# cvg/pixel-perfect-sfm

Hardware: AMD Instinct MI355X
Metric: featuremetric residuals+Jacobians evaluated/sec (1M obs) (higher is better)
Workload: dtype f32 horizontal / f64 vertical+normalisation on f16 patches; 1 GPU; BASELINE.json configs[2]: synthetic 200 cams / 200000 points / 1000000 obs featuremetric BA residual+Jacobian evaluation, 128-ch fp16 16x16 patches, SIMPLE_RADIAL, fused six-scalar Jacobian reduction; n_obs=1000000, channels=128, patch=16, obs_per_gpu=1000000, partition=none

## Files before the change

### pixel-perfect-sfm_amd/csrc/pxr_ba_solve.hip

```cpp
#include <hip/hip_runtime.h>

#include <algorithm>
#include <chrono>
#include <cmath>
#include <cstdlib>
#include <cstring>
#include <limits>
#include <thread>
#include <vector>

#include "pxr_ba_pcg.h"
#include "pxr_ba_solve.h"
#include "pxr_device.h"
#include "pxr_internal.h"

namespace pxr {


constexpr int JAC_THREADS = 128;

__global__ __launch_bounds__(JAC_THREADS) void k_jac(const SolveDev d, const double* __restrict__ rec,
                                                     pxr_loss loss, double* __restrict__ L, double* __restrict__ W) {
  extern __shared__ double jstage[];
  const int lane = threadIdx.x & 63, wave = threadIdx.x >> 6;
  const int LS = d.LS, W3 = 3 * d.DC, WS = W3 + 1;
  double* Lw = jstage + (size_t)wave * 64 * (LS + WS);
  double* Ww = Lw + (size_t)64 * LS;
  const int64_t i0 = (int64_t)blockIdx.x * blockDim.x + wave * 64;
  const int64_t i = i0 + lane;
  const int n_valid = (int)min((int64_t)64, d.v.n_obs - i0);
  if (i < d.v.n_obs) {
  const int img = d.v.d_obs_image[i], pt = d.v.d_obs_point[i], cam = d.v.d_image_camera[img];
  double q[4], t[3], X[3], k[PXR_KPAD];
#pragma unroll
  for (int j = 0; j < 4; ++j) q[j] = d.v.d_qvec[4 * (size_t)img + j];
#pragma unroll
  for (int j = 0; j < 3; ++j) { t[j] = d.v.d_tvec[3 * (size_t)img + j]; X[j] = d.v.d_xyz[3 * (size_t)pt + j]; }
#pragma unroll
  for (int j = 0; j < PXR_KPAD; ++j) k[j] = d.v.d_cam_params[(size_t)cam * PXR_KPAD + j];
  const int model = d.v.d_cam_model[cam];
  double x, y, A[2][3], Pq[2][4], PX[2][3], Pk[2][PXR_KPAD];
  world_to_pixel_jac(model, k, q, t, X, x, y, A, Pq, PX, Pk);

  const double* r = rec + (size_t)i * PXR_OBS_REC;
  const double s = r[0], gxx = r[1], gxy = r[2], gyy = r[3], bx = r[4], by = r[5];
  double rho[3];
  loss_eval(loss.type, loss.a, 1.0, s, rho);
  double kappa = 0.0;
  if (s != 0.0 && rho[2] > 0.0) {
    const double D = 1.0 + 2.0 * s * rho[2] / rho[1];
    const double alpha = 1.0 - sqrt(D);
    kappa = (2.0 * alpha - alpha * alpha) / s;
  }
  double* Lo = Lw + (size_t)lane * LS;
  const double m00 = rho[1] * (gxx - kappa * bx * bx), m01 = rho[1] * (gxy - kappa * bx * by),
               m11 = rho[1] * (gyy - kappa * by * by);
  Lo[0] = m00; Lo[1] = m01; Lo[2] = m11;
  Lo[3] = rho[1] * bx;
  Lo[4] = rho[1] * by;
  const bool pvar = d.pt_var[pt] != 0;
  double e0[3], e1[3];
#pragma unroll
  for (int j = 0; j < 3; ++j) {
    const double sc = pvar ? d.scale_p[3 * (size_t)pt + j] : 0.0;
    e0[j] = PX[0][j] * sc; e1[j] = PX[1][j] * sc;
    Lo[5 + j] = e0[j];
    Lo[8 + j] = e1[j];
  }
  double me0[3], me1[3];
#pragma unroll
  for (int j = 0; j < 3; ++j) {
    me0[j] = m00 * e0[j] + m01 * e1[j];
    me1[j] = m01 * e0[j] + m11 * e1[j];
  }
  double* Wo = Ww + (size_t)lane * WS;
  double* B0 = Lo + 11;
  double* B1 = B0 + d.DC;
  int col = 0;
  auto put = [&](int c, double b0, double b1) {
    B0[c] = b0; B1[c] = b1;
    Wo[3 * c] = b0 * me0[0] + b1 * me1[0];
    Wo[3 * c + 1] = b0 * me0[1] + b1 * me1[1];
    Wo[3 * c + 2] = b0 * me0[2] + b1 * me1[2];
  };
  if (d.pose_dim[img] > 0) {
    const int po = d.pose_off[img];
    const double PJ[4][3] = {{-q[1], -q[2], -q[3]}, {q[0], q[3], -q[2]}, {-q[3], q[0], q[1]}, {q[2], -q[1], q[0]}};
#pragma unroll
    for (int a = 0; a < 3; ++a) {
      const double sc = d.scale_c[po + a];
      put(col, (Pq[0][0] * PJ[0][a] + Pq[0][1] * PJ[1][a] + Pq[0][2] * PJ[2][a] + Pq[0][3] * PJ[3][a]) * sc,
          (Pq[1][0] * PJ[0][a] + Pq[1][1] * PJ[1][a] + Pq[1][2] * PJ[2][a] + Pq[1][3] * PJ[3][a]) * sc);
      ++col;
    }
    const int tm = d.tmask[img];
#pragma unroll
    for (int a = 0; a < 3; ++a) {
      if ((tm >> a) & 1) continue;
      const double sc = d.scale_c[po + col];
      put(col, A[0][a] * sc, A[1][a] * sc);
      ++col;
    }
  }
  if (d.intr_dim[cam] > 0) {
    const int io = d.intr_off[cam], cm = d.cmask[cam], K = camera_num_params(model);
    int kc = 0;
#pragma unroll
    for (int a = 0; a < PXR_KPAD; ++a) {
      if (a >= K || ((cm >> a) & 1)) continue;
      const double sc = d.scale_c[io + kc];
      put(col, Pk[0][a] * sc, Pk[1][a] * sc);
      ++col; ++kc;
    }
  }
  for (; col < d.DC; ++col) put(col, 0.0, 0.0);
  }
  __threadfence_block();
  __builtin_amdgcn_wave_barrier();
  if (n_valid <= 0) return;
  double* Lg = L + (size_t)i0 * LS;
  for (int x = lane; x < n_valid * LS; x += 64) Lg[x] = Lw[x];
  double* Wg = W + (size_t)i0 * W3;
  for (int x = lane; x < n_valid * W3; x += 64) { const int o = x / W3; Wg[x] = Ww[o * WS + (x - o * W3)]; }
}

__global__ __launch_bounds__(256) void k_point(const SolveDev d, const int64_t* __restrict__ pt_ptr,
                                               const int64_t* __restrict__ pt_obs,
                                               const double* __restrict__ L, double* __restrict__ V,
                                               double* __restrict__ gp) {
  const int64_t p = (int64_t)blockIdx.x * blockDim.x + threadIdx.x;
  if (p >= d.v.n_points) return;
  double v[6] = {0, 0, 0, 0, 0, 0}, g[3] = {0, 0, 0};
  for (int64_t o = pt_ptr[p]; o < pt_ptr[p + 1]; ++o) {
    const double* Lo = L + (size_t)pt_obs[o] * d.LS;
    const double m00 = Lo[0], m01 = Lo[1], m11 = Lo[2], b0 = Lo[3], b1 = Lo[4];
    const double e0[3] = {Lo[5], Lo[6], Lo[7]}, e1[3] = {Lo[8], Lo[9], Lo[10]};
    double me0[3], me1[3];
#pragma unroll
    for (int j = 0; j < 3; ++j) { me0[j] = m00 * e0[j] + m01 * e1[j]; me1[j] = m01 * e0[j] + m11 * e1[j]; }
    v[0] += e0[0] * me0[0] + e1[0] * me1[0];
    v[1] += e0[0] * me0[1] + e1[0] * me1[1];
    v[2] += e0[0] * me0[2] + e1[0] * me1[2];
    v[3] += e0[1] * me0[1] + e1[1] * me1[1];
    v[4] += e0[1] * me0[2] + e1[1] * me1[2];
    v[5] += e0[2] * me0[2] + e1[2] * me1[2];
#pragma unroll
    for (int j = 0; j < 3; ++j) g[j] += e0[j] * b0 + e1[j] * b1;
  }
#pragma unroll
  for (int j = 0; j < 6; ++j) V[6 * p + j] = v[j];
#pragma unroll
  for (int j = 0; j < 3; ++j) gp[3 * p + j] = g[j];
}

constexpr int IMG_BATCH = 128;

__global__ __launch_bounds__(256) void k_img(const SolveDev d, const ImgChunk* __restrict__ chunks,
                                             const int64_t* __restrict__ img_obs,
                                             const double* __restrict__ L, double* __restrict__ U,
                                             double* __restrict__ gc, int block_form, double det_scale,
                                             double* __restrict__ chunk_trace, double* __restrict__ kpart, int ne_max) {
  extern __shared__ double stage[];
  const ImgChunk ch = chunks[blockIdx.x];
  const int img = ch.img, cam = d.v.d_image_camera[img];
  const int dc = d.pose_dim[img] + d.intr_dim[cam];
  if (dc == 0) { if (threadIdx.x == 0 && chunk_trace) chunk_trace[blockIdx.x] = 0.0; return; }
  const int LS = d.LS;
  double* red = stage + (size_t)IMG_BATCH * LS;
  const int NP = dc * (dc + 1) / 2, NE = NP + dc;
  const int slices = 256 / NE;
  const int e = threadIdx.x % NE, sl = threadIdx.x / NE;
  int a = 0, b = 0;
  const bool is_g = e >= NP;
  if (is_g) { a = e - NP; }
  else { int rem = e; a = 0; while (rem >= dc - a) { rem -= dc - a; ++a; } b = a + rem; }
  double acc = 0.0;
  long long qacc = 0;
  const bool fixed = det_scale != 0.0;
  constexpr int IMG_PF = 16;
  double pf[IMG_PF];
  auto request = [&](int64_t base) {
    const int nb = (int)min((int64_t)IMG_BATCH, ch.end - base);
#pragma unroll
    for (int j = 0; j < IMG_PF; ++j) {
      const int x = threadIdx.x + 256 * j;
      const int xc = min(x, nb * LS - 1);
      const int o = xc / LS, f = xc - o * LS;
      pf[j] = L[(size_t)img_obs[base + o] * LS + f];
    }
  };
  if (LS <= 2 * IMG_PF) {
    if (ch.begin < ch.end) request(ch.begin);
    for (int64_t base = ch.begin; base < ch.end; base += IMG_BATCH) {
      const int nb = (int)min((int64_t)IMG_BATCH, ch.end - base);
#pragma unroll
      for (int j = 0; j < IMG_PF; ++j) { const int x = threadIdx.x + 256 * j; if (x < nb * LS) stage[x] = pf[j]; }
      __syncthreads();
      if (base + IMG_BATCH < ch.end) request(base + IMG_BATCH);
      if (sl < slices) {
        for (int o = sl; o < nb; o += slices) {
          const double* Lo = stage + (size_t)o * LS;
          const double* B0 = Lo + 11; const double* B1 = B0 + d.DC;
          const double term = is_g ? B0[a] * Lo[3] + B1[a] * Lo[4]
                                   : B0[a] * (Lo[0] * B0[b] + Lo[1] * B1[b]) + B1[a] * (Lo[1] * B0[b] + Lo[2] * B1[b]);
          acc += term;
          if (fixed) qacc += __double2ll_rn(term * det_scale);
        }
      }
      __syncthreads();
    }
  } else {
  for (int64_t base = ch.begin; base < ch.end; base += IMG_BATCH) {
    const int nb = (int)min((int64_t)IMG_BATCH, ch.end - base);
    for (int x = threadIdx.x; x < nb * LS; x += 256) {
      const int o = x / LS, f = x - o * LS;
      stage[x] = L[(size_t)img_obs[base + o] * LS + f];
    }
    __syncthreads();
    if (sl < slices) {
      for (int o = sl; o < nb; o += slices) {
        const double* Lo = stage + (size_t)o * LS;
        const double* B0 = Lo + 11; const double* B1 = B0 + d.DC;
        const double term = is_g ? B0[a] * Lo[3] + B1[a] * Lo[4]
                                 : B0[a] * (Lo[0] * B0[b] + Lo[1] * B1[b]) + B1[a] * (Lo[1] * B0[b] + Lo[2] * B1[b]);
        acc += term;
        if (fixed) qacc += __double2ll_rn(term * det_scale);
      }
    }
    __syncthreads();
  }
  }
  red[threadIdx.x] = acc;
  __syncthreads();
  if (sl == 0) for (int s2 = 1; s2 < slices; ++s2) acc += red[s2 * NE + e];
  if (fixed) {
    __syncthreads();
    red[threadIdx.x] = __longlong_as_double(qacc);
    __syncthreads();
    if (sl == 0) for (int s2 = 1; s2 < slices; ++s2) qacc += __double_as_longlong(red[s2 * NE + e]);
    __syncthreads();
    red[threadIdx.x] = (sl == 0 && !is_g && a == b) ? acc : 0.0;
    __syncthreads();
    if (threadIdx.x == 0 && chunk_trace) {
      double tr = 0.0;
      for (int x = 0; x < NP; ++x) tr += red[x];
      chunk_trace[blockIdx.x] = tr;
    }
  }
  if (sl == 0 && kpart) {
    kpart[(size_t)blockIdx.x * ne_max + e] = acc;
  } else if (sl == 0) {
    const int ra = col_index(d, img, cam, a);
    const double v = fixed ? __longlong_as_double(qacc) : acc;
    if (is_g) accum_flush(gc + ra, v, det_scale);
    else if (block_form) {
      double* Ub = U + (size_t)img * d.DC * d.DC;
      accum_flush(Ub + a * d.DC + b, v, det_scale);
      if (a != b) accum_flush(Ub + b * d.DC + a, v, det_scale);
    } else accum_flush(U + (size_t)ra * d.n_c + col_index(d, img, cam, b), v, det_scale);
  }
}

__global__ __launch_bounds__(256) void k_pinv(int64_t n_points, const int* __restrict__ pt_var,
                                              const double* __restrict__ V,
                                              const double* __restrict__ Vdiag0 ,
                                              double inv_radius, double* __restrict__ T,
                                              double* __restrict__ zero_ptr, int zero_n) {
  if (blockIdx.x == 0) for (int e = threadIdx.x; e < zero_n; e += blockDim.x) zero_ptr[e] = 0.0;
  const int64_t p = (int64_t)blockIdx.x * blockDim.x + threadIdx.x;
  if (p >= n_points) return;
  double* To = T + 6 * p;
  if (!pt_var[p]) { for (int j = 0; j < 6; ++j) To[j] = 0.0; return; }
  const double a00 = V[6 * p] + Vdiag0[3 * p] * inv_radius, a01 = V[6 * p + 1], a02 = V[6 * p + 2];
  const double a11 = V[6 * p + 3] + Vdiag0[3 * p + 1] * inv_radius, a12 = V[6 * p + 4];
  const double a22 = V[6 * p + 5] + Vdiag0[3 * p + 2] * inv_radius;
  const double c00 = a11 * a22 - a12 * a12, c01 = a02 * a12 - a01 * a22, c02 = a01 * a12 - a02 * a11;
  const double det = a00 * c00 + a01 * c01 + a02 * c02;
  const double id = 1.0 / det;
  To[0] = c00 * id; To[1] = c01 * id; To[2] = c02 * id;
  To[3] = (a00 * a22 - a02 * a02) * id; To[4] = (a01 * a02 - a00 * a12) * id;
  To[5] = (a00 * a11 - a01 * a01) * id;
}

struct Copy4 { const double* src[4]; double* dst[4]; int64_t n[4]; };
__global__ __launch_bounds__(256) void k_copy4(const Copy4 c) {
  const int64_t stride = (int64_t)gridDim.x * blockDim.x, t0 = (int64_t)blockIdx.x * blockDim.x + threadIdx.x;
#pragma unroll
  for (int a = 0; a < 4; ++a)
    for (int64_t e = t0; e < c.n[a]; e += stride) c.dst[a][e] = c.src[a][e];
}

__global__ __launch_bounds__(256) void k_schur(const SolveDev d, const int64_t* __restrict__ pt_ptr,
                                               const int64_t* __restrict__ pt_obs,
                                               const double* __restrict__ W, const double* __restrict__ T,
                                               const double* __restrict__ gp, double* __restrict__ S,
                                               double* __restrict__ rhs, double det_scale) {
  const int64_t tid = (int64_t)blockIdx.x * blockDim.x + threadIdx.x;
  const int64_t i = tid / d.DC;
  const int a = (int)(tid - i * d.DC);
  if (i >= d.v.n_obs) return;
  const int img = d.v.d_obs_image[i], cam = d.v.d_image_camera[img];
  const int dci = d.pose_dim[img] + d.intr_dim[cam];
  if (a >= dci) return;
  const int pt = d.v.d_obs_point[i];
  if (!d.pt_var[pt]) return;
  double y0, y1, y2;
  y_row(W, T, i, a, d.DC, pt, y0, y1, y2);
  const int r = col_index(d, img, cam, a);
  accum_add(rhs + (size_t)r * d.ldS, -(y0 * gp[3 * (size_t)pt] + y1 * gp[3 * (size_t)pt + 1] + y2 * gp[3 * (size_t)pt + 2]), det_scale);
  for (int64_t o = pt_ptr[pt]; o < pt_ptr[pt + 1]; ++o) {
    const int64_t j = pt_obs[o];
    const int imgj = d.v.d_obs_image[j], camj = d.v.d_image_camera[imgj];
    const int dcj = d.pose_dim[imgj] + d.intr_dim[camj];
    const double* Wj = W + (size_t)j * d.DC * 3;
    for (int b = 0; b < dcj; ++b) {
      const int c = col_index(d, imgj, camj, b);
      if (r > c) continue;
      accum_add(S + (size_t)r * d.ldS + c, -(y0 * Wj[3 * b] + y1 * Wj[3 * b + 1] + y2 * Wj[3 * b + 2]), det_scale);
    }
  }
}

template <int G>
__global__ __launch_bounds__(1024) void k_schur_lds(const SolveDev d, const ImgChunk* __restrict__ chunks,
                                                    const int4* __restrict__ so,
                                                    const int* __restrict__ pj,
                                                    const int4* __restrict__ pcols,
                                                    const double* __restrict__ W, const double* __restrict__ T,
                                                    const double* __restrict__ gp, int CT,
                                                    double* __restrict__ S, double* __restrict__ rhs, double det_scale) {
  extern __shared__ double acc[];
  const ImgChunk ch = chunks[blockIdx.x];
  const int img = ch.img, cam = d.v.d_image_camera[img];
  const int dci = d.pose_dim[img] + d.intr_dim[cam];
  if (dci == 0) return;
  const int c0 = blockIdx.y * CT, c1 = min(d.n_c, c0 + CT);
  double* racc = acc + (size_t)d.DC * CT;
  double* ybuf = racc + d.DC;
  for (int e = threadIdx.x; e < dci * CT + d.DC; e += blockDim.x) {
    if (e < dci * CT) acc[(e / CT) * CT + (e % CT)] = 0.0; else racc[e - dci * CT] = 0.0;
  }
  __syncthreads();
  const int lane_b = threadIdx.x % G, grp = threadIdx.x / G, n_grp = blockDim.x / G;
  int rrow[G];
#pragma unroll
  for (int a = 0; a < G; ++a) rrow[a] = a < dci ? col_index(d, img, cam, a) : 0x7fffffff;
  constexpr int PB = 8;
  const bool first_tile = blockIdx.y == 0;
  int64_t o = ch.begin + grp;
  int4 s = o < ch.end ? so[o] : make_int4(0, 0, 0, 0);
  while (o < ch.end) {
    const int64_t o_next = o + n_grp;
    const int4 s_next = o_next < ch.end ? so[o_next] : make_int4(0, 0, 0, 0);
    if (s.w != 0) {
      const int64_t i = s.x, pt = s.y;
      const bool row_ok = lane_b < dci;
      const double* Wi = W + ((size_t)i * d.DC + (row_ok ? lane_b : 0)) * 3;
      const double* Tp = T + 6 * (size_t)pt;
      const double* gpp = gp + 3 * (size_t)pt;
      const double w0 = Wi[0], w1 = Wi[1], w2 = Wi[2];
      const double t0 = Tp[0], t1 = Tp[1], t2 = Tp[2], t3 = Tp[3], t4 = Tp[4], t5 = Tp[5];
      const double g0 = gpp[0], g1 = gpp[1], g2 = gpp[2];
      double y0 = 0.0, y1 = 0.0, y2 = 0.0;
      for (int kb = 0; kb < s.w; kb += PB) {
        int jj[PB];
        int4 cc[PB];
#pragma unroll
        for (int u = 0; u < PB; ++u) {
          const int idx = s.z + min(kb + u, s.w - 1);
          jj[u] = pj[idx]; cc[u] = pcols[idx];
        }
        double mm[PB][3];
        int col[PB];
#pragma unroll
        for (int u = 0; u < PB; ++u) {
          const int pdj = cc[u].y, dcj = pdj + cc[u].w;
          const bool has = kb + u < s.w && lane_b < dcj;
          const double* Wj = W + ((size_t)jj[u] * d.DC + (has ? lane_b : 0)) * 3;
          mm[u][0] = Wj[0]; mm[u][1] = Wj[1]; mm[u][2] = Wj[2];
          const int c = lane_b < pdj ? cc[u].x + lane_b : cc[u].z + (lane_b - pdj);
          col[u] = (has && c >= c0 && c < c1) ? c : -1;
        }
        if (kb == 0) {
          if (row_ok) { y0 = w0 * t0 + w1 * t1 + w2 * t2; y1 = w0 * t1 + w1 * t3 + w2 * t4; y2 = w0 * t2 + w1 * t4 + w2 * t5; }
          if (first_tile && row_ok) accum_add(racc + lane_b, -(y0 * g0 + y1 * g1 + y2 * g2), det_scale);
          double* yb = ybuf + 3 * (size_t)threadIdx.x;
          yb[0] = y0; yb[1] = y1; yb[2] = y2;
        }
        const double* yg = ybuf + 3 * (size_t)(threadIdx.x - lane_b);
#pragma unroll
        for (int a = 0; a < G; ++a) {
          const double ya0 = yg[3 * a], ya1 = yg[3 * a + 1], ya2 = yg[3 * a + 2];
#pragma unroll
          for (int u = 0; u < PB; ++u) {
            const int c = col[u];
            if (c >= 0 && c >= rrow[a])
              accum_add(acc + (size_t)a * CT + (c - c0), -(ya0 * mm[u][0] + ya1 * mm[u][1] + ya2 * mm[u][2]), det_scale);
          }
        }
      }
    }
    o = o_next; s = s_next;
  }
  __syncthreads();
  for (int e = threadIdx.x; e < dci * CT; e += blockDim.x) {
    const int a = e / CT, cl = e % CT;
    const double v = acc[(size_t)a * CT + cl];
    if (__double_as_longlong(v) != 0ll) accum_flush(S + (size_t)col_index(d, img, cam, a) * d.ldS + (c0 + cl), v, det_scale);
  }
  if (blockIdx.y == 0 && threadIdx.x < dci) {
    const double v = racc[threadIdx.x];
    if (__double_as_longlong(v) != 0ll) accum_flush(rhs + (size_t)col_index(d, img, cam, threadIdx.x) * d.ldS, v, det_scale);
  }
}

__global__ void k_copy_upper_add_diag(int n, const double* __restrict__ U, const double* __restrict__ damp,
                                      double inv_radius, const double* __restrict__ gc, double* __restrict__ S,
                                      int add_u, double det_scale) {
  const int64_t t = (int64_t)blockIdx.x * blockDim.x + threadIdx.x;
  const int ld = n + 1;
  if (t >= (int64_t)n * ld) return;
  const int r = (int)(t / ld), c = (int)(t % ld);
  double v = S[t];
  if (add_u) {
    v = (c < n && r <= c) ? U[(size_t)r * n + c] : 0.0;
  }
  else {
    if (det_scale != 0.0) v = (double)__double_as_longlong(v) / det_scale;
    if (r == c) v += damp[r] * inv_radius;
    if (c == n) v += gc[r];
  }
  S[t] = v;
}

__global__ void k_extract_diag(int n, const double* __restrict__ U, double* __restrict__ out) {
  const int i = blockIdx.x * blockDim.x + threadIdx.x;
  if (i < n) out[i] = U[(size_t)i * n + i];
}

__global__ void k_clamp(int64_t n, const double* __restrict__ in, double lo, double hi, double* __restrict__ out) {
  const int64_t i = (int64_t)blockIdx.x * blockDim.x + threadIdx.x;
  if (i < n) out[i] = fmin(fmax(in[i], lo), hi);
}

__global__ void k_point_diag(int64_t n_points, const double* __restrict__ V, double* __restrict__ out) {
  const int64_t p = (int64_t)blockIdx.x * blockDim.x + threadIdx.x;
  if (p >= n_points) return;
  out[3 * p] = V[6 * p]; out[3 * p + 1] = V[6 * p + 3]; out[3 * p + 2] = V[6 * p + 5];
}

__global__ void k_jacobi_scale(int64_t n, const double* __restrict__ diag, double* __restrict__ scale) {
  const int64_t i = (int64_t)blockIdx.x * blockDim.x + threadIdx.x;
  if (i < n) scale[i] = 1.0 / (1.0 + sqrt(diag[i]));
}

__global__ void k_axpy1(int n, const double* __restrict__ x, double* __restrict__ y) {
  const int i = blockIdx.x * blockDim.x + threadIdx.x;
  if (i < n) y[i] += x[i];
}

__global__ void k_fill(int64_t n, double v, double* __restrict__ out) {
  const int64_t i = (int64_t)blockIdx.x * blockDim.x + threadIdx.x;
  if (i < n) out[i] = v;
}

__global__ void k_finish_camera_step(int n, const double* __restrict__ x, const double* __restrict__ gc,
                                     const double* __restrict__ damp, double inv_radius,
                                     double* __restrict__ delta_c, double* __restrict__ scal_rep, long long* __restrict__ limb) {
  __shared__ long long lsh[PXR_LIMBS * 4];
  const int i = blockIdx.x * blockDim.x + threadIdx.x;
  double part = 0.0;
  if (i < n) {
    const double dl = -x[i];
    delta_c[i] = dl;
    part = dl * (damp[i] * inv_radius * dl - gc[i]);
  }
  if (limb) {
    Limbs l;
    if (i < n) l.add(part);
    limbs_block_add(l, limb + (8 + 0) * PXR_LIMBS, lsh);
// ... 799 lines not shown
    if (ctx->rank != 0) hipLaunchKernelGGL(k_zero, dim3(nblk(count)), dim3(256), 0, st, count, buf);
    return ar(buf, count);
  };
  struct { long long* p; } slimb;
  slimb.p = reinterpret_cast<long long*>(scal.p + 16);
  long long* const limb_arg = det ? slimb.p : nullptr;
  DevBuf<double> i64_halves;
  const bool native_i64 = allreduce == nullptr;
  if (det && multi && !native_i64) RC(i64_halves.alloc((size_t)2 * std::max<int64_t>({packed_doubles, 2 * (int64_t)nc1 + 8, 16 * PXR_LIMBS})));
  auto ar_i64 = [&](long long* buf, int64_t count) -> int {
    if (!multi || count <= 0) return PXR_OK;
    if (native_i64) return comm_allreduce_sum_i64(ctx, buf, count);
    hipLaunchKernelGGL(k_i64_split, dim3(nblk(count)), dim3(256), 0, st, count, (const long long*)buf, i64_halves.p);
    RC(ar(i64_halves.p, 2 * count));
    hipLaunchKernelGGL(k_i64_join, dim3(nblk(count)), dim3(256), 0, st, count, (const double*)i64_halves.p, buf);
    return PXR_OK;
  };
  auto zero_scalars = [&]() -> int {
    PXR_HIP(hipMemsetAsync(scal.p, 0, sizeof(double) * (16 + 16 * PXR_LIMBS + 1), st));
    return PXR_OK;
  };
  struct { double* p; } lin_stats;
  constexpr int kScalAll = 16 + 16 * PXR_LIMBS + 1 + 4;
  lin_stats.p = scal.p + (kScalAll - 4);
  if (!ctx->h_readback) PXR_HIP(hipHostMalloc(&ctx->h_readback, 4096, hipHostMallocDefault));
  static_assert(sizeof(double) * kScalAll <= 4096, "read-back buffer");
  double* const h_scal = static_cast<double*>(ctx->h_readback);
  std::memset(h_scal, 0, sizeof(double) * kScalAll);
  double* const h_lin_stats = h_scal + (kScalAll - 4);
  const int* const h_info_word = reinterpret_cast<const int*>(h_scal + 16 + 16 * PXR_LIMBS);
  const bool spin_wait = std::getenv("PXR_BLOCKING_WAIT") == nullptr;
  auto read_scal = [&](double* h16) -> int {
    if (det) {
      RC(ar_i64(slimb.p, 8 * PXR_LIMBS));
      hipLaunchKernelGGL(k_limbs_finish, dim3(1), dim3(64), 0, st, (const long long*)slimb.p, 0xffffu, scal.p);
    } else {
      hipLaunchKernelGGL(k_limbs_finish, dim3(1), dim3(64), 0, st, (const long long*)slimb.p, (1u << 0) | (1u << 4), scal.p);
      RC(ar(scal_sum, 8));
      RC(from_rank0(scal_rep, 8));
    }
    PXR_HIP(hipMemcpyAsync(h_scal, scal.p, sizeof(double) * kScalAll, hipMemcpyDeviceToHost, st));
    if (spin_wait) {
      PXR_HIP(hipEventRecord(ctx->ev_sync, st));
      hipError_t q;
      while ((q = hipEventQuery(ctx->ev_sync)) == hipErrorNotReady) {}
      PXR_HIP(q);
    } else PXR_HIP(hipStreamSynchronize(st));
    std::memcpy(h16, h_scal, sizeof(double) * 16);
    return PXR_OK;
  };
  DevBuf<double> det_part, chunk_trace;
  RC(det_part.alloc((size_t)n_pts + 8));
  RC(chunk_trace.alloc(chunks.size() + 1));
  auto det_scale_for = [](double md, double cost_now) {
    const double bound = 8.0 * std::max({md, std::sqrt(2.0 * md * std::max(cost_now, 0.0)), 1e-300});
    return std::ldexp(1.0, 62 - (int)std::ceil(std::log2(bound)));
  };
  double lin_md = 1.0;
  bool gram_cache = !geom && ctx->gram_cache && gram_eval_supported(arena, view) && cfg->use_float_simd == 0;
  bool gram_inner = !geom && opt->use_inner_iterations != 0 && arena->dtype != PXR_F64 && (arena->C == 128 || arena->C == 64) && !getenv("PXR_INNER_OLD") &&
                    !getenv("PXR_INNER_PACKED") && cfg->use_float_simd == 0;
  for (int c = 0; c < n_cam; ++c) gram_inner = gram_inner && cam_model[c] <= PXR_OPENCV;
  bool inner_cache = gram_inner && gram_eval_supported(arena, view) && !getenv("PXR_INNER_NO_CACHE");
  GramCache gram;
  if ((gram_cache || inner_cache) && gram_eval_prepare(ctx, arena, view, &gram) != PXR_OK) {
    gram_cache = false; inner_cache = false;
    (void)set_error(PXR_OK, "");
  }
  bool geom_ext = false;
  for (int c = 0; c < n_cam; ++c) geom_ext = geom_ext || cam_model[c] > PXR_OPENCV;
  setup_mark("Gram-matrix cache prepared");
  bool gram_warm = false;
  int n_evaluations = 0;
  bool cur_is_exact = true;
  auto evaluate = [&](const pxr_ba_view& v, double* rec) -> int {
    if (geom) RC(geom_eval(ctx, &v, d_obs_xy, rec, nullptr));
    else if (gram_cache && n_evaluations > 0) { RC(gram_evaluate(ctx, arena, &v, cfg, gram, rec)); gram_warm = true; }
    else RC(ba_eval_with_cost(ctx, arena, &v, cfg, 1, rec, nullptr, nullptr, nullptr, nullptr, nullptr));
    ++n_evaluations;
    hipLaunchKernelGGL(k_cost_limbs, dim3(1024), dim3(256), 0, st, (const double*)rec, n_obs, *loss, slimb.p + 0 * PXR_LIMBS);
    LAUNCH_CHECK("cost");
    return PXR_OK;
  };
  double lin_scale = 0.0;
  auto linearize = [&](const double* rec) -> int {
    hipLaunchKernelGGL(k_jac, dim3((unsigned)((n_obs + JAC_THREADS - 1) / JAC_THREADS)), dim3(JAC_THREADS),
                       sizeof(double) * (JAC_THREADS / 64) * 64 * (LS + 3 * DC + 1), st, dv, rec, *loss, L.p, W.p);
    hipLaunchKernelGGL(k_point, dim3(nblk(n_pts)), dim3(256), 0, st, dv, d_pt_ptr.p, d_pt_obs.p, L.p, V.p, gp.p);
    PXR_HIP(hipMemsetAsync(U.p, 0, sizeof(double) * U.n, st));
    PXR_HIP(hipMemsetAsync(gcd.p, 0, sizeof(double) * gcd.n, st));
    if (n_c > 0 && !chunks.empty()) {
      hipLaunchKernelGGL(k_img, dim3((unsigned)chunks.size()), dim3(256), sizeof(double) * ((size_t)IMG_BATCH * LS + 256), st, dv,
                         d_chunks.p, d_img_obs.p, L.p, U.p, gc, iterative ? 1 : 0, lin_scale, lin_scale != 0.0 ? chunk_trace.p : (double*)nullptr,
                         det_iter ? det_kpart.p : (double*)nullptr, det_ne_max);
      if (det_iter) {
        RC(pcg_blocks_from_partials(st, dv, d_kchunk_ptr.p, det_kpart.p, det_ne_max, U.p, det_gimg.p, d_col_ent_ptr.p, d_col_ent.p, diagU, gc));
        LAUNCH_CHECK("linearize kernels");
        RC(ar(gcd.p, 2 * (int64_t)nc1));
        return PXR_OK;
      }
      if (lin_scale != 0.0) {
        hipLaunchKernelGGL(k_diag_and_trace, dim3(1), dim3(1024), 0, st, n_c, (const double*)U.p, diagU, (const double*)chunk_trace.p, (int)chunks.size(),
                           reinterpret_cast<long long*>(gcd.p + 2 * nc1));
        RC(ar_i64(reinterpret_cast<long long*>(gcd.p), 2 * (int64_t)nc1 + PXR_LIMBS));
        hipLaunchKernelGGL(k_finish_and_stats, dim3(1), dim3(1024), 0, st, n_c, 2 * (int)nc1, gcd.p, lin_scale,
                           reinterpret_cast<const long long*>(gcd.p + 2 * nc1), lin_stats.p);
        LAUNCH_CHECK("linearize kernels");
        return PXR_OK;
      }
      if (iterative) RC(pcg_diag_from_blocks(st, dv, U.p, diagU));
      else hipLaunchKernelGGL(k_extract_diag, dim3(nblk(n_c)), dim3(256), 0, st, n_c, U.p, diagU);
    }
    LAUNCH_CHECK("linearize kernels");
    RC(ar(gcd.p, 2 * (int64_t)nc1));
    return PXR_OK;
  };
  auto lin_fits = [&](const double* stt, double md_made_for) {
    if (n_c == 0 || chunks.empty()) return true;
    const double mx = stt[0], sm = stt[1], mn = stt[2], tr = stt[3];
    if (!(std::isfinite(mx) && std::isfinite(sm) && std::isfinite(tr))) return false;
    if (mn < 0.0) return false;
    if (std::fabs(tr - sm) > std::ldexp(1.0, 61) / lin_scale) return false;
    return mx <= 8.0 * md_made_for;
  };
  bool lin_not_finite = false;
  auto linearize_checked = [&](const double* rec, double md_guess, double cost_now, bool refine = false) -> int {
    if (!det_fixed) return linearize(rec);
    for (int attempt = 0; attempt < 8; ++attempt) {
      lin_md = md_guess;
      lin_scale = det_scale_for(lin_md, cost_now);
      RC(linearize(rec));
      PXR_HIP(hipMemcpyAsync(h_lin_stats, lin_stats.p, sizeof(double) * 4, hipMemcpyDeviceToHost, st));
      PXR_HIP(hipStreamSynchronize(st));
      if (lin_fits(h_lin_stats, lin_md)) {
        if (refine && attempt == 0 && h_lin_stats[0] * 64.0 < md_guess) { md_guess = std::max(h_lin_stats[0], 1e-300); continue; }
        return PXR_OK;
      }
      if (!(std::isfinite(h_lin_stats[3]) && h_lin_stats[3] >= 0.0)) { lin_not_finite = true; return PXR_OK; }
      md_guess = std::max(h_lin_stats[3], 2.0 * md_guess);
    }
    return set_error(PXR_EINVAL, "pxr_ba_solve: the fixed-point grid of the deterministic mode could not be fitted");
  };
  auto refresh_damping = [&]() -> int {
    if (n_c > 0) hipLaunchKernelGGL(k_clamp, dim3(nblk(n_c)), dim3(256), 0, st, (int64_t)n_c, diagU, opt->min_lm_diagonal, opt->max_lm_diagonal, damp_c.p);
    hipLaunchKernelGGL(k_point_diag, dim3(nblk(n_pts)), dim3(256), 0, st, n_pts, V.p, Vd0.p);
    hipLaunchKernelGGL(k_clamp, dim3(nblk(n_pts * 3)), dim3(256), 0, st, n_pts * 3, Vd0.p, opt->min_lm_diagonal, opt->max_lm_diagonal, Vd0.p);
    LAUNCH_CHECK("damping kernels");
    return PXR_OK;
  };

  if (iterative) {
    pcg.st = st; pcg.dv = dv;
    pcg.chunks = d_schur_chunks.p; pcg.n_chunks = (int)schur_chunks.size(); pcg.so = d_so.p;
    pcg.pt_ptr = d_pt_ptr.p; pcg.part_obs = d_part_obs.p; pcg.obs_cols = d_obs_cols.p;
    pcg.W = W.p; pcg.T = T.p; pcg.gp = gp.p; pcg.gc = gc; pcg.damp_c = damp_c.p; pcg.Ublk = U.p;
    pcg.n_groups = (int)group_size.size(); pcg.col_group = d_col_group.p; pcg.group_size = d_group_size.p;
    pcg.group_cols = d_group_cols.p;
    pcg.u = pcg_u.p; pcg.Mloc = pcg_mloc.p; pcg.Gm = pcg_g.p;
    pcg.x = xsol.p; pcg.r = pcg_vec.p; pcg.p = pcg_vec.p + nc1; pcg.q = pcg_vec.p + 2 * nc1; pcg.z = pcg_vec.p + 3 * nc1;
    pcg.b = pcg_vec.p + 4 * nc1; pcg.cgs = pcg_scal.p; pcg.cg_part = pcg_scal.p + 16; pcg.d_fail = d_info;
    pcg.det = det_iter;
    if (det_iter) {
      pcg.chunk_ptr = d_schunk_ptr.p; pcg.col_ent_ptr = d_col_ent_ptr.p; pcg.col_ent = d_col_ent.p;
      pcg.wpart = det_wpart.p; pcg.mpart = det_mpart.p;
    }
  }
  const std::function<int(double*, int64_t)> ar_fn = ar;
  auto gradient_below_tolerance = [&](bool* below) -> int {
    double h[16];
    RC(zero_scalars());
    if (n_c > 0) hipLaunchKernelGGL(k_count_above, dim3(nblk(n_c)), dim3(256), 0, st, (int64_t)n_c, gc, scale_c.p, opt->gradient_tolerance, scal_rep + 4,
                                    det ? slimb.p + (8 + 4) * PXR_LIMBS : (long long*)nullptr);
    hipLaunchKernelGGL(k_count_above, dim3(nblk(n_pts * 3)), dim3(256), 0, st, n_pts * 3, gp.p, scale_p.p, opt->gradient_tolerance, scal_sum + 5,
                       det ? slimb.p + 5 * PXR_LIMBS : (long long*)nullptr);
    RC(read_scal(h));
    *below = h[5] == 0.0 && h[12] == 0.0;
    return PXR_OK;
  };

  struct InnerListsOwner { InnerLists l; ~InnerListsOwner() { free_inner_lists(&l); } } inner_lists;
  if (gram_inner) {
    const int64_t* h_pt_ptr = pt_cnt.data();
    std::vector<int64_t> pageable;
    void* wave_stage = nullptr;
    const size_t ptr_bytes = (sizeof(int64_t) * ((size_t)n_pts + 1) + 255) & ~(size_t)255, wave_bytes = inner_wave_stage_bytes(n_pts);
    if (device_lists) {
      int64_t* stage = (ptr_bytes + wave_bytes) <= ((size_t)1 << 28) ? static_cast<int64_t*>(setup_staging(ctx, ptr_bytes + wave_bytes)) : nullptr;
      if (stage) wave_stage = reinterpret_cast<char*>(stage) + ptr_bytes;
      else { pageable.resize((size_t)n_pts + 1); stage = pageable.data(); }
      PXR_HIP(hipMemcpyAsync(stage, d_pt_ptr.p, sizeof(int64_t) * ((size_t)n_pts + 1), hipMemcpyDeviceToHost, st));
      PXR_HIP(hipStreamSynchronize(st));
      h_pt_ptr = stage;
    }
    RC(make_inner_lists(ctx, h_pt_ptr, n_pts, wave_stage, wave_stage ? wave_bytes : 0, view, d_pt_ptr.p, d_pt_obs.p, &inner_lists.l));
  }
  setup_mark("inner-iteration tables");
  const auto t_loop0 = std::chrono::steady_clock::now();
  sum->setup_ms = std::chrono::duration<double, std::milli>(t_loop0 - t_setup0).count();
  sum->num_camera_unknowns = n_c; sum->num_point_unknowns = 3 * n_pvar;
  sum->iterations = 0; sum->num_successful = 0; sum->termination = PXR_TERM_NO_CONVERGENCE;
  const bool use_lds_schur = std::getenv("PXR_SCHUR_GLOBAL_ATOMICS") == nullptr;
  int CT = n_c > 0 ? std::min(n_c, (int)((128 * 1024 / 8 - DC) / DC)) : 1;
  int n_ctiles = n_c > 0 ? (n_c + CT - 1) / CT : 1;
  if (const char* e = std::getenv("PXR_SCHUR_CTILES")) n_ctiles = std::max(n_ctiles, std::min(std::max(1, n_c), std::atoi(e)));
  CT = n_c > 0 ? (n_c + n_ctiles - 1) / n_ctiles : 1;
  const size_t schur_shmem = sizeof(double) * ((size_t)DC * CT + DC + 3 * 1024);
  if (use_lds_schur && n_c > 0)
    PXR_HIP(hipFuncSetAttribute(reinterpret_cast<const void*>(DC <= 8 ? k_schur_lds<8> : (DC <= 16 ? k_schur_lds<16> : k_schur_lds<32>)),
                                hipFuncAttributeMaxDynamicSharedMemorySize, (int)schur_shmem));
  PXR_HIP(hipFuncSetAttribute(reinterpret_cast<const void*>(k_jac), hipFuncAttributeMaxDynamicSharedMemorySize,
                              (int)(sizeof(double) * (JAC_THREADS / 64) * 64 * (LS + 3 * DC + 1))));
  const bool verbose = std::getenv("PXR_VERBOSE") != nullptr;
  const bool phase_timing = std::getenv("PXR_PHASE_TIMING") != nullptr;
  double ph_ms[8] = {0, 0, 0, 0, 0, 0, 0, 0};
  auto ph_t0 = std::chrono::steady_clock::now();
  auto phase = [&](int k) {
    if (!phase_timing) return;
    (void)hipStreamSynchronize(st);
    const auto now = std::chrono::steady_clock::now();
    ph_ms[k] += std::chrono::duration<double, std::milli>(now - ph_t0).count();
    ph_t0 = now;
  };

  double hs[16];
  double* rec_cur = rec_a.p; double* rec_cand = rec_b.p;
  RC(zero_scalars());
  RC(evaluate(dv.v, rec_cur));
  RC(read_scal(hs));
  double cost = hs[0];
  sum->initial_cost = cost;
  if (!std::isfinite(cost)) {
    sum->final_cost = cost; sum->termination = PXR_TERM_FAILURE;
    sum->total_ms = std::chrono::duration<double, std::milli>(std::chrono::steady_clock::now() - t_loop0).count();
    return PXR_OK;
  }
  hipLaunchKernelGGL(k_fill, dim3(nblk(nc1)), dim3(256), 0, st, (int64_t)nc1, 1.0, scale_c.p);
  hipLaunchKernelGGL(k_fill, dim3(nblk(n_pts * 3)), dim3(256), 0, st, n_pts * 3, 1.0, scale_p.p);
  RC(linearize_checked(rec_cur, std::ldexp(1.0, 32), cost, !opt->jacobi_scaling));
  auto fail_not_finite = [&]() -> int {
    sum->final_cost = cost; sum->final_radius = opt->initial_radius; sum->termination = PXR_TERM_FAILURE;
    sum->total_ms = std::chrono::duration<double, std::milli>(std::chrono::steady_clock::now() - t_loop0).count();
    return PXR_OK;
  };
  if (lin_not_finite) return fail_not_finite();
  if (opt->jacobi_scaling) {
    if (n_c > 0) hipLaunchKernelGGL(k_jacobi_scale, dim3(nblk(n_c)), dim3(256), 0, st, (int64_t)n_c, diagU, scale_c.p);
    hipLaunchKernelGGL(k_point_diag, dim3(nblk(n_pts)), dim3(256), 0, st, n_pts, V.p, Vd0.p);
    hipLaunchKernelGGL(k_jacobi_scale, dim3(nblk(n_pts * 3)), dim3(256), 0, st, n_pts * 3, Vd0.p, scale_p.p);
    RC(linearize_checked(rec_cur, 1.0 / 8.0, cost));
    if (lin_not_finite) return fail_not_finite();
  }
  if (opt->gradient_tolerance > 0.0) {
    bool below = false;
    RC(gradient_below_tolerance(&below));
    if (below) {
      sum->termination = PXR_TERM_CONVERGENCE; sum->final_cost = cost; sum->final_radius = opt->initial_radius;
      sum->total_ms = std::chrono::duration<double, std::milli>(std::chrono::steady_clock::now() - t_loop0).count();
      return PXR_OK;
    }
  }
  double radius = opt->initial_radius, decrease_factor = 2.0;
  int invalid = 0;
  bool reuse_diag = false;
  bool inner_enabled = opt->use_inner_iterations != 0, inner_useful = false;
  PXR_HIP(hipStreamSynchronize(st));
  sum->initial_us = (int32_t)std::min<double>(2e9, 1e3 * std::chrono::duration<double, std::milli>(std::chrono::steady_clock::now() - t_loop0).count());
  bool any_cb = ctx->iter_cb != nullptr;
  if (multi) {
    double h = any_cb ? 1.0 : 0.0;
    PXR_HIP(hipMemcpyAsync(cb_flags.p, &h, sizeof(h), hipMemcpyHostToDevice, st));
    RC(ar(cb_flags.p, 1));
    PXR_HIP(hipMemcpyAsync(&h, cb_flags.p, sizeof(h), hipMemcpyDeviceToHost, st));
    PXR_HIP(hipStreamSynchronize(st));
    any_cb = h > 0.0;
  }
  auto notify = [&](int iteration, bool valid, bool successful, double cost_now, double change, double rel, double radius_next, double step) -> int {
    if (!any_cb) return 0;
    int rc = 0;
    if (ctx->iter_cb) {
      pxr_iteration_summary is;
      is.iteration = iteration; is.step_is_valid = valid; is.step_is_successful = successful; is.cost = cost_now; is.cost_change = change;
      is.relative_decrease = rel; is.trust_region_radius = radius_next; is.step_norm = step;
      rc = ctx->iter_cb(&is, ctx->iter_user);
    }
    if (multi) {
      double h[2] = {rc == 1 ? 1.0 : 0.0, rc == 2 ? 1.0 : 0.0};
      if (hipMemcpyAsync(cb_flags.p, h, sizeof(h), hipMemcpyHostToDevice, st) != hipSuccess || ar(cb_flags.p, 2) != PXR_OK ||
          hipMemcpyAsync(h, cb_flags.p, sizeof(h), hipMemcpyDeviceToHost, st) != hipSuccess || hipStreamSynchronize(st) != hipSuccess)
        return 1;
      rc = h[0] > 0.0 ? 1 : (h[1] > 0.0 ? 2 : 0);
    }
    return rc;
  };
  auto user_stop = [&](int rc) {
    if (rc == 1) { sum->termination = PXR_TERM_FAILURE; return true; }
    if (rc == 2) { sum->termination = PXR_TERM_CONVERGENCE; return true; }
    return false;
  };
  if (user_stop(notify(0, false, false, cost, 0.0, 0.0, radius, 0.0))) {
    sum->final_cost = cost; sum->final_radius = radius;
    sum->total_ms = std::chrono::duration<double, std::milli>(std::chrono::steady_clock::now() - t_loop0).count();
    return PXR_OK;
  }

  while (true) {
    if (sum->iterations >= opt->max_iterations) { sum->termination = PXR_TERM_NO_CONVERGENCE; break; }
    if (radius < opt->min_radius) { sum->termination = PXR_TERM_CONVERGENCE; break; }
    ++sum->iterations;
    phase(7);
    if (!reuse_diag) RC(refresh_damping());
    const double inv_radius = 1.0 / radius;
    hipLaunchKernelGGL(k_pinv, dim3(nblk(n_pts)), dim3(256), 0, st, n_pts, d_pt_var.p, V.p, Vd0.p, inv_radius, T.p, scal.p, 16 + 16 * PXR_LIMBS + 1);
    if (n_pts == 0) RC(zero_scalars());
    bool ok = true;
    double inexact_correction = 0.0;
    if (n_c > 0 && iterative) {
      PcgResult pr;
      RC(pcg_solve(pcg, inv_radius, opt, ar_fn, &pr));
      phase(2);
      sum->linear_iterations += pr.iterations;
      if (!pr.ok) ok = false;
      inexact_correction = 0.5 * pr.x_dot_r;
      PXR_HIP(hipMemsetAsync(d_info, 0, sizeof(int), st));
      hipLaunchKernelGGL(k_finish_camera_step, dim3(nblk(n_c)), dim3(256), 0, st, n_c, xsol.p, gc, damp_c.p, inv_radius, delta_c.p, scal_rep, limb_arg);
      RC(from_rank0(delta_c.p, n_c));
    } else if (n_c > 0) {
      const double schur_scale = det_fixed ? lin_scale : 0.0;
      hipLaunchKernelGGL(k_copy_upper_add_diag, dim3(nblk((int64_t)n_c * ldS)), dim3(256), 0, st, n_c, U.p, (const double*)nullptr, 0.0, (const double*)nullptr, S.p, 1, schur_scale);
      if (use_lds_schur) {
#define SCHUR_LAUNCH(GG)                                                                                              \
  hipLaunchKernelGGL(k_schur_lds<GG>, dim3((unsigned)schur_chunks.size(), (unsigned)n_ctiles), dim3(1024), schur_shmem, st, dv, \
                     d_schur_chunks.p, d_so.p, d_part_obs.p, d_obs_cols.p, W.p, T.p, gp.p, CT, S.p, rhs, schur_scale)
        if (DC <= 8) SCHUR_LAUNCH(8); else if (DC <= 16) SCHUR_LAUNCH(16); else SCHUR_LAUNCH(32);
#undef SCHUR_LAUNCH
      } else {
        hipLaunchKernelGGL(k_schur, dim3(nblk(n_obs * DC)), dim3(256), 0, st, dv, d_pt_ptr.p, d_pt_obs.p, W.p, T.p, gp.p, S.p, rhs, schur_scale);
      }
      LAUNCH_CHECK("schur kernels");
      phase(0);
      if (multi) {
        hipLaunchKernelGGL(k_pack_upper, dim3((unsigned)n_c), dim3(256), 0, st, n_c, S.p, S_packed.p);
        if (schur_scale != 0.0) RC(ar_i64(reinterpret_cast<long long*>(S_packed.p), packed_doubles));
        else RC(ar(S_packed.p, packed_doubles));
        hipLaunchKernelGGL(k_unpack_upper, dim3((unsigned)n_c), dim3(256), 0, st, n_c, S_packed.p, S.p);
        LAUNCH_CHECK("pack / unpack of the reduced camera system");
      }
      phase(1);
      hipLaunchKernelGGL(k_copy_upper_add_diag, dim3(nblk((int64_t)n_c * ldS)), dim3(256), 0, st, n_c, U.p, damp_c.p, inv_radius, gc, S.p, 0, schur_scale);
      RC(chol_factor_solve(st, S.p, n_c, d_info, linv.p, xsol.p, false));
      phase(2);
      hipLaunchKernelGGL(k_finish_camera_step, dim3(nblk(n_c)), dim3(256), 0, st, n_c, xsol.p, gc, damp_c.p, inv_radius, delta_c.p, scal_rep, limb_arg);
      RC(from_rank0(delta_c.p, n_c));
    }
    phase(3);
    double model_cost_change = 0, cand_cost = 0, step_norm = 0, x_norm = 0;
    if (ok) {
#define BACKSUB_LAUNCH(GG)                                                                                                          \
  hipLaunchKernelGGL(k_backsub<GG>, dim3(nblk((n_pts * GG + BACKSUB_PPG - 1) / BACKSUB_PPG)), dim3(256), 0, st, dv, d_pt_ptr.p, d_part_obs.p, d_obs_cols.p, W.p, T.p, gp.p, \
                     delta_c.p, Vd0.p, inv_radius, delta_p.p, scal_sum, limb_arg)
      if (DC <= 8) BACKSUB_LAUNCH(8); else if (DC <= 16) BACKSUB_LAUNCH(16); else BACKSUB_LAUNCH(32);
#undef BACKSUB_LAUNCH
      ParamPtrs out{q1.p, t1.p, k1.p, X1.p};
      const int64_t upd_blocks = nblk(((int64_t)n_img + n_cam + n_pts + UPDATE_IPT - 1) / UPDATE_IPT);
      hipLaunchKernelGGL(k_update, dim3((unsigned)upd_blocks), dim3(256), 0, st, dv, delta_c.p, delta_p.p, out, scal_rep, scal_sum, limb_arg);
      LAUNCH_CHECK("step kernels");
      const bool do_inner = inner_enabled;
      if (do_inner) {
        PXR_HIP(hipMemsetAsync(det_part.p, 0, sizeof(double) * (size_t)n_pts, st));
        if (geom) RC(launch_inner_geom(ctx, &cand_view, d_obs_xy, loss, d_pt_ptr.p, d_pt_obs.p, d_pt_var.p, scal_sum + 4, det_part.p, geom_ext));
        else {
          RC(launch_inner_iterations(ctx, arena, &cand_view, cfg, loss, d_pt_ptr.p, d_pt_obs.p, d_pt_var.p, scal_sum + 4, gram_inner ? &inner_lists.l : nullptr,
                                     det_part.p, (gram_cache || inner_cache) ? &gram : nullptr, gram_warm));
          gram_warm = true;
        }
        hipLaunchKernelGGL(k_limb_accumulate, dim3(256), dim3(256), 0, st, (const double*)det_part.p, n_pts, slimb.p + 4 * PXR_LIMBS);
        PXR_HIP(hipMemsetAsync(scal_sum + 2, 0, sizeof(double), st));
        PXR_HIP(hipMemsetAsync(slimb.p + 2 * PXR_LIMBS, 0, sizeof(long long) * PXR_LIMBS, st));
        hipLaunchKernelGGL(k_point_step_norm, dim3(nblk(n_pts)), dim3(256), 0, st, n_pts, d_pt_var.p, cur_X, X1.p, scal_sum + 2,
                           det ? slimb.p + 2 * PXR_LIMBS : (long long*)nullptr);
        LAUNCH_CHECK("inner iteration kernels");
      }
      phase(4);
      RC(evaluate(cand_view, rec_cand));
      RC(read_scal(hs));
      const int h_info = *h_info_word;
      if (det_fixed && !lin_fits(h_lin_stats, lin_md)) {
        RC(linearize_checked(rec_cur, std::max(h_lin_stats[3], 2.0 * lin_md), cost));
        if (lin_not_finite) { sum->termination = PXR_TERM_FAILURE; break; }
        --sum->iterations;
        continue;
      }
      if (n_c > 0 && h_info != 0) ok = false;
      phase(5);
      cand_cost = hs[0];
      model_cost_change = 0.5 * (hs[1] + hs[8]) + inexact_correction;
      step_norm = std::sqrt(hs[2] + hs[9]);
      x_norm = std::sqrt(hs[3] + hs[10]);
      if (!(model_cost_change > 0.0) || !std::isfinite(model_cost_change)) ok = false;
      if (!std::isfinite(cand_cost)) cand_cost = std::numeric_limits<double>::max();
      inner_useful = false;
      if (ok && do_inner && cand_cost < std::numeric_limits<double>::max()) {
        const double cost_before = hs[4];
        model_cost_change += cost_before - cand_cost;
        inner_useful = cand_cost < cost;
        inner_enabled = (1.0 - cand_cost / cost_before) > opt->inner_iteration_tolerance;
      }
    }
    if (verbose)
      fprintf(stderr, "[pxr_ba_solve] it %3d cost %.9e cand %.9e mcc %.3e radius %.3e |dx| %.3e %s\n", sum->iterations,
              cost, cand_cost, model_cost_change, radius, step_norm, ok ? "" : "INVALID");
    auto reevaluate_current = [&]() -> int {
      if (!(gram_cache && cur_is_exact && n_evaluations > 1)) return PXR_OK;
      double h2[16];
      RC(zero_scalars());
      RC(evaluate(dv.v, rec_cur));
      RC(read_scal(h2));
      if (std::isfinite(h2[0])) cost = h2[0];
// ... 73 lines not shown
```

Measured before the change: 1.425 billion residual_blocks/s.

## Specialise Schur LDS kernel on fixed-point mode and skip inactive rows via masks

Adds a fast magic-number fixed-point rounding helper with a wave-uniform fallback to the slow conversion when values exceed a safe limit, and uses it in k_img and the Schur kernel. The Schur LDS kernel is templated on whether fixed-point accumulation is used, and per-lane column/row comparisons are replaced by ballot-derived row bitmasks so rows with no active updates are skipped. These changes target the BA solve's Schur and image accumulation kernels, not the Jacobian evaluation the metric counts. They add template instantiations and ballot overhead.

```diff
diff --git a/pixel-perfect-sfm_amd/csrc/pxr_ba_solve.hip b/pixel-perfect-sfm_amd/csrc/pxr_ba_solve.hip
--- a/pixel-perfect-sfm_amd/csrc/pxr_ba_solve.hip
+++ b/pixel-perfect-sfm_amd/csrc/pxr_ba_solve.hip
@@ -12,6 +12,7 @@
 #include "pxr_ba_pcg.h"
 #include "pxr_ba_solve.h"
 #include "pxr_device.h"
+#include "pxr_fixed_point.h"
 #include "pxr_internal.h"
 
 namespace pxr {
@@ -158,7 +159,7 @@
 __global__ __launch_bounds__(256) void k_img(const SolveDev d, const ImgChunk* __restrict__ chunks,
                                              const int64_t* __restrict__ img_obs,
                                              const double* __restrict__ L, double* __restrict__ U,
-                                             double* __restrict__ gc, int block_form, double det_scale,
+                                             double* __restrict__ gc, int block_form, double det_scale, double fx_limit,
                                              double* __restrict__ chunk_trace, double* __restrict__ kpart, int ne_max) {
   extern __shared__ double stage[];
   const ImgChunk ch = chunks[blockIdx.x];
@@ -204,7 +205,7 @@
           const double term = is_g ? B0[a] * Lo[3] + B1[a] * Lo[4]
                                    : B0[a] * (Lo[0] * B0[b] + Lo[1] * B1[b]) + B1[a] * (Lo[1] * B0[b] + Lo[2] * B1[b]);
           acc += term;
-          if (fixed) qacc += __double2ll_rn(term * det_scale);
+          if (fixed) qacc += fx_round(term, det_scale, fx_limit);
         }
       }
       __syncthreads();
@@ -224,7 +225,7 @@
         const double term = is_g ? B0[a] * Lo[3] + B1[a] * Lo[4]
                                  : B0[a] * (Lo[0] * B0[b] + Lo[1] * B1[b]) + B1[a] * (Lo[1] * B0[b] + Lo[2] * B1[b]);
         acc += term;
-        if (fixed) qacc += __double2ll_rn(term * det_scale);
+        if (fixed) qacc += fx_round(term, det_scale, fx_limit);
       }
     }
     __syncthreads();
@@ -321,19 +322,31 @@
   }
 }
 
-template <int G>
+template <bool FIXED>
+__device__ __forceinline__ void schur_add(double* slot, double v, bool active, double det_scale, double fx_limit) {
+  if constexpr (FIXED) {
+    const long long q = fx_round(v, det_scale, fx_limit, active);
+    if (active) atomicAdd(reinterpret_cast<unsigned long long*>(slot), (unsigned long long)q);
+  } else {
+    if (active) atomicAdd(slot, v);
+  }
+}
+
+template <int G, bool FIXED>
 __global__ __launch_bounds__(1024) void k_schur_lds(const SolveDev d, const ImgChunk* __restrict__ chunks,
                                                     const int4* __restrict__ so,
                                                     const int* __restrict__ pj,
                                                     const int4* __restrict__ pcols,
                                                     const double* __restrict__ W, const double* __restrict__ T,
                                                     const double* __restrict__ gp, int CT,
-                                                    double* __restrict__ S, double* __restrict__ rhs, double det_scale) {
+                                                    double* __restrict__ S, double* __restrict__ rhs, double det_scale,
+                                                    double fx_limit) {
   extern __shared__ double acc[];
   const ImgChunk ch = chunks[blockIdx.x];
   const int img = ch.img, cam = d.v.d_image_camera[img];
-  const int dci = d.pose_dim[img] + d.intr_dim[cam];
+  const int pd_i = d.pose_dim[img], id_i = d.intr_dim[cam], dci = pd_i + id_i;
   if (dci == 0) return;
+  const int po_i = d.pose_off[img], io_i = d.intr_off[cam];
   const int c0 = blockIdx.y * CT, c1 = min(d.n_c, c0 + CT);
   double* racc = acc + (size_t)d.DC * CT;
   double* ybuf = racc + d.DC;
@@ -342,9 +355,7 @@
   }
   __syncthreads();
   const int lane_b = threadIdx.x % G, grp = threadIdx.x / G, n_grp = blockDim.x / G;
-  int rrow[G];
-#pragma unroll
-  for (int a = 0; a < G; ++a) rrow[a] = a < dci ? col_index(d, img, cam, a) : 0x7fffffff;
+  const unsigned pose_rows = (1u << pd_i) - 1u, intr_rows = ((dci >= 32 ? 0u : (1u << dci)) - 1u) & ~pose_rows;
   constexpr int PB = 8;
   const bool first_tile = blockIdx.y == 0;
   int64_t o = ch.begin + grp;
@@ -371,7 +382,10 @@
           jj[u] = pj[idx]; cc[u] = pcols[idx];
         }
         double mm[PB][3];
-        int col[PB];
+        int off[PB];
+        int na[PB];
+        unsigned rows[PB];
+        unsigned rows_any = 0u;
 #pragma unroll
         for (int u = 0; u < PB; ++u) {
           const int pdj = cc[u].y, dcj = pdj + cc[u].w;
@@ -379,23 +393,30 @@
           const double* Wj = W + ((size_t)jj[u] * d.DC + (has ? lane_b : 0)) * 3;
           mm[u][0] = Wj[0]; mm[u][1] = Wj[1]; mm[u][2] = Wj[2];
           const int c = lane_b < pdj ? cc[u].x + lane_b : cc[u].z + (lane_b - pdj);
-          col[u] = (has && c >= c0 && c < c1) ? c : -1;
+          const int n = min(max(c - po_i + 1, 0), pd_i) + min(max(c - io_i + 1, 0), id_i);
+          na[u] = (has && c >= c0 && c < c1) ? n : 0;
+          off[u] = c - c0;
+          rows[u] = (__builtin_amdgcn_ballot_w64(na[u] > 0) != 0ull ? pose_rows : 0u) |
+                    (__builtin_amdgcn_ballot_w64(na[u] > pd_i) != 0ull ? intr_rows : 0u);
+          rows_any |= rows[u];
         }
         if (kb == 0) {
           if (row_ok) { y0 = w0 * t0 + w1 * t1 + w2 * t2; y1 = w0 * t1 + w1 * t3 + w2 * t4; y2 = w0 * t2 + w1 * t4 + w2 * t5; }
-          if (first_tile && row_ok) accum_add(racc + lane_b, -(y0 * g0 + y1 * g1 + y2 * g2), det_scale);
+          schur_add<FIXED>(racc + lane_b, -(y0 * g0 + y1 * g1 + y2 * g2), first_tile && row_ok, det_scale, fx_limit);
           double* yb = ybuf + 3 * (size_t)threadIdx.x;
           yb[0] = y0; yb[1] = y1; yb[2] = y2;
         }
         const double* yg = ybuf + 3 * (size_t)(threadIdx.x - lane_b);
 #pragma unroll
         for (int a = 0; a < G; ++a) {
-          const double ya0 = yg[3 * a], ya1 = yg[3 * a + 1], ya2 = yg[3 * a + 2];
-#pragma unroll
-          for (int u = 0; u < PB; ++u) {
-            const int c = col[u];
-            if (c >= 0 && c >= rrow[a])
-              accum_add(acc + (size_t)a * CT + (c - c0), -(ya0 * mm[u][0] + ya1 * mm[u][1] + ya2 * mm[u][2]), det_scale);
+          if ((rows_any >> a) & 1u) {
+            const double ya0 = yg[3 * a], ya1 = yg[3 * a + 1], ya2 = yg[3 * a + 2];
+            double* arow = acc + (size_t)a * CT;
+#pragma unroll
+            for (int u = 0; u < PB; ++u) {
+              if ((rows[u] >> a) & 1u)
+                schur_add<FIXED>(arow + off[u], -(ya0 * mm[u][0] + ya1 * mm[u][1] + ya2 * mm[u][2]), a < na[u], det_scale, fx_limit);
+            }
           }
         }
       }
@@ -1361,6 +1382,8 @@
     LAUNCH_CHECK("cost");
     return PXR_OK;
   };
+  const char* const schur_convert = std::getenv("PXR_SCHUR_CONVERT");
+  const bool fx_force_slow = schur_convert != nullptr && std::strcmp(schur_convert, "slow") == 0;
   double lin_scale = 0.0;
   auto linearize = [&](const double* rec) -> int {
     hipLaunchKernelGGL(k_jac, dim3((unsigned)((n_obs + JAC_THREADS - 1) / JAC_THREADS)), dim3(JAC_THREADS),
@@ -1370,7 +1393,7 @@
     PXR_HIP(hipMemsetAsync(gcd.p, 0, sizeof(double) * gcd.n, st));
     if (n_c > 0 && !chunks.empty()) {
       hipLaunchKernelGGL(k_img, dim3((unsigned)chunks.size()), dim3(256), sizeof(double) * ((size_t)IMG_BATCH * LS + 256), st, dv,
-                         d_chunks.p, d_img_obs.p, L.p, U.p, gc, iterative ? 1 : 0, lin_scale, lin_scale != 0.0 ? chunk_trace.p : (double*)nullptr,
+                         d_chunks.p, d_img_obs.p, L.p, U.p, gc, iterative ? 1 : 0, lin_scale, fx_fast_limit(lin_scale, fx_force_slow), lin_scale != 0.0 ? chunk_trace.p : (double*)nullptr,
                          det_iter ? det_kpart.p : (double*)nullptr, det_ne_max);
       if (det_iter) {
         RC(pcg_blocks_from_partials(st, dv, d_kchunk_ptr.p, det_kpart.p, det_ne_max, U.p, det_gimg.p, d_col_ent_ptr.p, d_col_ent.p, diagU, gc));
@@ -1484,9 +1507,16 @@
   if (const char* e = std::getenv("PXR_SCHUR_CTILES")) n_ctiles = std::max(n_ctiles, std::min(std::max(1, n_c), std::atoi(e)));
   CT = n_c > 0 ? (n_c + n_ctiles - 1) / n_ctiles : 1;
   const size_t schur_shmem = sizeof(double) * ((size_t)DC * CT + DC + 3 * 1024);
+  using SchurLdsFn = void (*)(const SolveDev, const ImgChunk*, const int4*, const int*, const int4*, const double*, const double*,
+                              const double*, int, double*, double*, double, double);
+  auto schur_lds_fn = [DC](bool fixed) -> SchurLdsFn {
+    if (DC <= 8) return fixed ? k_schur_lds<8, true> : k_schur_lds<8, false>;
+    if (DC <= 16) return fixed ? k_schur_lds<16, true> : k_schur_lds<16, false>;
+    return fixed ? k_schur_lds<32, true> : k_schur_lds<32, false>;
+  };
   if (use_lds_schur && n_c > 0)
-    PXR_HIP(hipFuncSetAttribute(reinterpret_cast<const void*>(DC <= 8 ? k_schur_lds<8> : (DC <= 16 ? k_schur_lds<16> : k_schur_lds<32>)),
-                                hipFuncAttributeMaxDynamicSharedMemorySize, (int)schur_shmem));
+    for (const bool fixed : {false, true})
+      PXR_HIP(hipFuncSetAttribute(reinterpret_cast<const void*>(schur_lds_fn(fixed)), hipFuncAttributeMaxDynamicSharedMemorySize, (int)schur_shmem));
   PXR_HIP(hipFuncSetAttribute(reinterpret_cast<const void*>(k_jac), hipFuncAttributeMaxDynamicSharedMemorySize,
                               (int)(sizeof(double) * (JAC_THREADS / 64) * 64 * (LS + 3 * DC + 1))));
   const bool verbose = std::getenv("PXR_VERBOSE") != nullptr;
@@ -1607,11 +1637,9 @@
       const double schur_scale = det_fixed ? lin_scale : 0.0;
       hipLaunchKernelGGL(k_copy_upper_add_diag, dim3(nblk((int64_t)n_c * ldS)), dim3(256), 0, st, n_c, U.p, (const double*)nullptr, 0.0, (const double*)nullptr, S.p, 1, schur_scale);
       if (use_lds_schur) {
-#define SCHUR_LAUNCH(GG)                                                                                              \
-  hipLaunchKernelGGL(k_schur_lds<GG>, dim3((unsigned)schur_chunks.size(), (unsigned)n_ctiles), dim3(1024), schur_shmem, st, dv, \
-                     d_schur_chunks.p, d_so.p, d_part_obs.p, d_obs_cols.p, W.p, T.p, gp.p, CT, S.p, rhs, schur_scale)
-        if (DC <= 8) SCHUR_LAUNCH(8); else if (DC <= 16) SCHUR_LAUNCH(16); else SCHUR_LAUNCH(32);
-#undef SCHUR_LAUNCH
+        hipLaunchKernelGGL(schur_lds_fn(schur_scale != 0.0), dim3((unsigned)schur_chunks.size(), (unsigned)n_ctiles), dim3(1024), schur_shmem, st, dv,
+                           d_schur_chunks.p, d_so.p, d_part_obs.p, d_obs_cols.p, W.p, T.p, gp.p, CT, S.p, rhs, schur_scale,
+                           fx_fast_limit(schur_scale, fx_force_slow));
       } else {
         hipLaunchKernelGGL(k_schur, dim3(nblk(n_obs * DC)), dim3(256), 0, st, dv, d_pt_ptr.p, d_pt_obs.p, W.p, T.p, gp.p, S.p, rhs, schur_scale);
       }
diff --git a/pixel-perfect-sfm_amd/csrc/pxr_fixed_point.h b/pixel-perfect-sfm_amd/csrc/pxr_fixed_point.h
--- /dev/null
+++ b/pixel-perfect-sfm_amd/csrc/pxr_fixed_point.h
@@ -0,0 +1,18 @@
+#pragma once
+#include <hip/hip_runtime.h>
+
+constexpr double PXR_FX_MAGIC = 6755399441055744.0;
+
+static inline double fx_fast_limit(double grid, bool force_slow) {
+  return (force_slow || !(grid > 0.0)) ? 0.0 : 2251799813685248.0 / grid;
+}
+
+__device__ __forceinline__ long long fx_round_slow(double v, double grid) { return __double2ll_rn(v * grid); }
+__device__ __forceinline__ long long fx_round_fast(double v, double grid) {
+  return __double_as_longlong(__fma_rn(v, grid, PXR_FX_MAGIC)) - __double_as_longlong(PXR_FX_MAGIC);
+}
+__device__ __forceinline__ long long fx_round(double v, double grid, double fast_limit, bool active = true) {
+  long long q = fx_round_fast(v, grid);
+  if (__builtin_expect(__builtin_amdgcn_ballot_w64(active && !(fabs(v) < fast_limit)) != 0ull, 0)) q = fx_round_slow(v, grid);
+  return q;
+}
```

Measured after the change: 1.425 billion residual_blocks/s, median of 2. No clear change (+0.1%).
